# sashajenner/honours

Measured on AMD Instinct MI355X. Metric: raw-signal MB/s (compress+decompress), higher is better.
Workload: dtype u16

## Files before the change

### honours_amd/csrc/press_huffman.hip

```cpp

#include "press_internal.h"
#include "press_packed.h"
#include <cstddef>
#include <type_traits>

namespace ph {

#ifdef HUF_STAMPS
__device__ unsigned long long g_hstamp[32];
#define HSTAMP_DECL                                             \
	unsigned long long hs_t = __builtin_amdgcn_s_memtime(); \
	unsigned long long hs_acc[8] = { 0, 0, 0, 0, 0, 0, 0, 0 }
#define HSTAMP(i)                                                              \
	do {     \
		__builtin_amdgcn_sched_barrier(0);                             \
		const unsigned long long hs_n = __builtin_amdgcn_s_memtime(); \
		hs_acc[(i) & 7] += hs_n - hs_t;                                \
		hs_t = hs_n;                                                   \
		__builtin_amdgcn_sched_barrier(0);                             \
	} while (0)
#define HSTAMP_FLUSH(base)                                                     \
	do {                                                                   \
		if ((threadIdx.x & 63) == 0)                                   \
			for (int hs_i = 0; hs_i < 8; hs_i++)                   \
				atomicAdd(&g_hstamp[(base) + hs_i], hs_acc[hs_i]); \
	} while (0)
#else
#define HSTAMP_DECL
#define HSTAMP(i)
#define HSTAMP_FLUSH(base)
#endif

constexpr uint32_t HEND = 0xFFFFFFFFu;
constexpr uint32_t R_END = 31;
constexpr int HT = HUF_HT;

__device__ __forceinline__ uint32_t uniform(uint32_t v) { return (uint32_t) __builtin_amdgcn_readfirstlane((int) v); }
__device__ __forceinline__ bool any64(bool c) { return __builtin_amdgcn_ballot_w64(c) != 0; }

__device__ __forceinline__ uint32_t wave_scan(uint32_t v)
{
	v += (uint32_t) __builtin_amdgcn_update_dpp(0, (int) v, 0x111, 0xf, 0xf, true);
	v += (uint32_t) __builtin_amdgcn_update_dpp(0, (int) v, 0x112, 0xf, 0xf, true);
	v += (uint32_t) __builtin_amdgcn_update_dpp(0, (int) v, 0x114, 0xf, 0xf, true);
	v += (uint32_t) __builtin_amdgcn_update_dpp(0, (int) v, 0x118, 0xf, 0xf, true);
	v += (uint32_t) __builtin_amdgcn_update_dpp(0, (int) v, 0x142, 0xa, 0xf, false);
	v += (uint32_t) __builtin_amdgcn_update_dpp(0, (int) v, 0x143, 0xc, 0xf, false);
	return v;
}

__device__ __noinline__ uint32_t trie_code(const HuffDev *hd, uint32_t wnd)
{
	int node = 0;
	uint32_t l = 0;
	while (node >= 0 && hd->leaf[node] < 0 && l < 32) {
		node = hd->child[node][(wnd >> l) & 1u];
		l++;
	}
	if (node < 0 || hd->leaf[node] < 0)
		return 0;
	return (uint32_t) hd->leaf[node] | (l << 8) | (l << 24);
}

template <int RU>
struct HufGeo {
	static constexpr int OWN = 2 * RU;
	static constexpr int NDW = OWN / 32 + 1;
	static constexpr int NCOL = NDW + 1;
};

__device__ __forceinline__ uint32_t clamp_nb(int64_t v)
{
	return v <= 0 ? 0u : (v > 0x7FFFFFFF ? 0x7FFFFFFFu : (uint32_t) v);
}

#ifndef HUF_NO_NT
__device__ __forceinline__ uint4 ld16_pay(const uint8_t *p)
{
	typedef uint32_t u32x4_u __attribute__((ext_vector_type(4), aligned(1)));
	const u32x4_u v = __builtin_nontemporal_load(reinterpret_cast<const u32x4_u *>(p));
	return make_uint4(v.x, v.y, v.z, v.w);
}
__device__ __forceinline__ uint32_t ld4_pay(const uint8_t *p)
{
	typedef uint32_t __attribute__((aligned(1))) u32_u;
	return __builtin_nontemporal_load(reinterpret_cast<const u32_u *>(p));
}
#else
__device__ __forceinline__ uint4 ld16_pay(const uint8_t *p)
{
	uint4 v;
	__builtin_memcpy(&v, p, 16);
	return v;
}
__device__ __forceinline__ uint32_t ld4_pay(const uint8_t *p)
{
	uint32_t v;
	__builtin_memcpy(&v, p, 4);
	return v;
}
#endif

template <int NDW, int S = 64>
__device__ __forceinline__ void col_load(uint32_t *col, const uint8_t *src, int32_t rb0, int32_t lo, int32_t nby)
{
	if (rb0 >= lo && rb0 + 4 * NDW <= nby) {
		const uint8_t *q = src + rb0;
		uint4 t[NDW / 4 ? NDW / 4 : 1];
		uint32_t x[NDW % 4 ? NDW % 4 : 1];
#pragma unroll
		for (int j = 0; j < NDW / 4; j++)
			t[j] = ld16_pay(q + 16 * j);
#pragma unroll
		for (int j = 0; j < NDW % 4; j++)
			x[j] = ld4_pay(q + 4 * (NDW / 4 * 4 + j));
#pragma unroll
		for (int j = 0; j < NDW / 4; j++) {
			col[(4 * j + 0) * S] = t[j].x;
			col[(4 * j + 1) * S] = t[j].y;
			col[(4 * j + 2) * S] = t[j].z;
			col[(4 * j + 3) * S] = t[j].w;
		}
#pragma unroll
		for (int j = 0; j < NDW % 4; j++)
			col[(NDW / 4 * 4 + j) * S] = x[j];
	} else if (nby > lo) {
		uint8_t b[4 * NDW];
#pragma unroll
		for (int i = 0; i < 4 * NDW; i++) {
			const int32_t r = rb0 + i;
			b[i] = src[r < lo ? lo : (r >= nby ? nby - 1 : r)];
		}
#pragma unroll
		for (int j = 0; j < NDW; j++) {
			uint32_t x = 0;
#pragma unroll
			for (int i = 0; i < 4; i++) {
				const int32_t r = rb0 + 4 * j + i;
				x |= (r >= lo && r < nby) ? (uint32_t) b[4 * j + i] << (8 * i) : 0u;
			}
			col[j * S] = x;
		}
	} else {
#pragma unroll
		for (int j = 0; j < NDW; j++)
			col[j * S] = 0;
	}
}

__device__ __forceinline__ int32_t unzz8(uint32_t z) { return (int32_t) (z >> 1) ^ -(int32_t) (z & 1u); }

typedef __attribute__((address_space(3))) const uint32_t *lds_cu32p;
typedef __attribute__((address_space(3))) const uint16_t *lds_cu16p;
typedef __attribute__((address_space(3))) const uint8_t *lds_cu8p;
typedef __attribute__((address_space(3))) uint8_t *lds_u8p;

struct LenTabs {
	alignas(16) uint32_t alut[1 << HUF_LUT_BITS];
	alignas(16) uint16_t flut[1 << HUF_LUT_BITS];
	alignas(16) uint16_t l2ld[HUF_L2_ENTRIES];
};

template <bool TRIE, int S = 64>
__device__ __forceinline__ uint32_t len_scan(const uint32_t *col_, const LenTabs *tabs, const HuffDev *hd, uint32_t start,
					     uint32_t lim, uint32_t nb, uint32_t &cnt, uint32_t &dsum)
{
	const lds_cu32p col = (lds_cu32p) col_;
	const lds_cu32p alut = (lds_cu32p) tabs->alut;
	const lds_cu16p flut = (lds_cu16p) tabs->flut;
	const lds_cu16p l2ld = (lds_cu16p) tabs->l2ld;
	bool bad = start == HEND;
	uint32_t L = lim < nb ? lim : nb;
	if (bad)
		L = 0;
	auto long_ld = [&](uint32_t e, uint32_t wnd) -> uint32_t {
		if (TRIE && e == 0xFFFFFFFFu) {
			const uint32_t t = trie_code(hd, wnd);
			return t ? (((t >> 24) & 31u) | (((uint32_t) unzz8(t & 0xFFu) & 0xFFu) << 8)) : 0u;
		}
		const uint32_t v = l2ld[(e & 0xFFFu) + ((wnd >> HUF_LUT_BITS) & ((1u << ((e >> 12) & 15u)) - 1u))];
		return v == 0xFFFFu ? 0u : v;
	};
	constexpr uint32_t PB = 30;
	const lds_cu32p colm = col - S;
	uint32_t A = (bad ? 0u : start) + PB;
	{
		int32_t LmP = (int32_t) L - HUF_LUT_BITS + (int32_t) PB;
		uint32_t jj = (A >> 5) & 15u;
		uint32_t w0 = colm[__umul24(jj, (uint32_t) S)], w1 = colm[__umul24(jj, (uint32_t) S) + S];
		while ((int32_t) (A & 0x1FFu) <= LmP) {
			const uint32_t pp = A & 0x1FFu;
			{
				const uint32_t w2 = colm[__umul24(jj, (uint32_t) S) + 2 * S];
				const uint32_t wnd = __builtin_amdgcn_alignbit(w1, w0, A);
				const uint32_t e = *(lds_cu32p) ((lds_cu8p) alut + (wnd & (((1u << HUF_LUT_BITS) - 1u) << 2)));
				uint32_t inc = e;
				if ((int32_t) e < 0) {
					const uint32_t ld = long_ld(e, wnd >> 2);
					const uint32_t tot = ld & 0xFFu;
					inc = tot | (1u << HUF_A_CNT) | (((uint32_t) (int32_t) (int8_t) (ld >> 8) & 0x7FFFu) << HUF_A_SUM);
					if (tot - 1u >= L + PB - pp) {
						inc = 0;
						LmP = -1;
					}
				}
				A += inc;
				const uint32_t jn = (A >> 5) & 15u;
				if (jn != jj) {
					w0 = w1;
					w1 = w2;
				}
				jj = jn;
			}
		}
	}
	uint32_t p = (A & 0x1FFu) - PB;
	uint32_t c = (A >> HUF_A_CNT) & 0x7Fu;
	int32_t d = (int32_t) (A << 1) >> 17;
	for (;;) {
		const bool act = p < L;
		if (!any64(act))
			break;
		const uint32_t pp = act ? p : 0u;
		const uint32_t j = pp >> 5;
		const int r0 = (int) __umul24(j, (uint32_t) S);
		const uint32_t wnd = __builtin_amdgcn_alignbit(col[r0 + S], col[r0], pp);
		const uint32_t e = alut[wnd & ((1u << HUF_LUT_BITS) - 1u)];
		const uint32_t f = flut[wnd & ((1u << HUF_LUT_BITS) - 1u)];
		uint32_t tot = e & 15u, n = (e >> HUF_A_CNT) & 15u, len1 = f & 0xFFu;
		int32_t dall = (int32_t) (e << 1) >> 17, d1 = (int32_t) (int8_t) (f >> 8);
		bool fail = false;
		if (any64(act && (int32_t) e < 0)) {
			if (act && (int32_t) e < 0) {
				const uint32_t ld = long_ld(e, wnd);
				tot = len1 = ld & 0xFFu;
				dall = d1 = (int32_t) (int8_t) (ld >> 8);
				fail = tot == 0;
				n = 1;
			}
		}
		const bool fits = pp + tot <= L;
		const bool cut = !fits && pp + len1 > nb;
		if (act && !fail && !cut) {
			p += fits ? tot : len1;
			c += fits ? n : 1u;
			d += fits ? dall : d1;
		}
		if (act && (fail || cut)) {
			bad = true;
			L = 0;
		}
	}
	cnt = c;
	dsum = (uint32_t) d & 0xFFFFu;
	return bad ? HEND : (p >= nb && p < lim ? HEND : p);
}

__device__ __forceinline__ void wave_lds_sync()
{
	__builtin_amdgcn_fence(__ATOMIC_RELEASE, "wavefront");
	__builtin_amdgcn_wave_barrier();
	__builtin_amdgcn_fence(__ATOMIC_ACQUIRE, "wavefront");
}



#ifndef HUF_SYNC_PER_CU
#define HUF_SYNC_PER_CU 2
#endif
#ifndef HUF_RUNUP_EIGHTHS
#define HUF_RUNUP_EIGHTHS 4
#endif
constexpr int WGS = 1024;
constexpr int SYNC_S = 64;

__device__ __forceinline__ uint32_t pack_rec(uint32_t f, uint32_t c, uint32_t d)
{
	return (f == HEND ? R_END : f) | ((c & 0xFFu) << 8) | ((d & 0xFFFFu) << 16);
}

constexpr uint32_t LIST_NONE = 0xFFFFFFFFu;
constexpr uint32_t SYNC_UC = 16;

__device__ __forceinline__ void list_push(uint32_t *list, uint32_t *cnt, uint32_t cap, bool yes, uint32_t value, uint32_t lane)
{
	const unsigned long long m = __ballot(yes);
	if (!m)
		return;
	uint32_t base = 0;
	if (lane == (uint32_t) __builtin_ctzll(m))
		base = atomicAdd(cnt, (uint32_t) __popcll(m));
	base = (uint32_t) __shfl((int) base, __builtin_ctzll(m), 64);
	const uint32_t idx = base + (uint32_t) __popcll(m & ((1ull << lane) - 1ull));
	if (yes && idx < cap)
		list[idx] = value;
}

__device__ __forceinline__ void load_len_tables(const HuffDev *hd, LenTabs *t, uint32_t nthr)
{
	const uint4 *s4 = reinterpret_cast<const uint4 *>(hd->alut);
	uint4 *d4 = reinterpret_cast<uint4 *>(t->alut);
	for (uint32_t i = threadIdx.x; i < (1u << HUF_LUT_BITS) / 4; i += nthr)
		d4[i] = s4[i];
	const uint4 *f4 = reinterpret_cast<const uint4 *>(hd->flut);
	uint4 *g4 = reinterpret_cast<uint4 *>(t->flut);
	for (uint32_t i = threadIdx.x; i < (1u << HUF_LUT_BITS) / 8; i += nthr)
		g4[i] = f4[i];
	const uint4 *t4 = reinterpret_cast<const uint4 *>(hd->l2ld);
	uint4 *u4 = reinterpret_cast<uint4 *>(t->l2ld);
	for (uint32_t i = threadIdx.x; i < (uint32_t) HUF_L2_ENTRIES / 8; i += nthr)
		u4[i] = t4[i];
}


template <int RU, bool TRIE>
__global__ __launch_bounds__(WGS, 2 * HUF_SYNC_PER_CU * 2) void k_huf_sync(DecodeArgs a)
{
	constexpr int OWN = HufGeo<RU>::OWN, NDW = HufGeo<RU>::NDW;
	constexpr int RUNUP = OWN * HUF_RUNUP_EIGHTHS / 8;
	constexpr int S = SYNC_S;
	struct Lds {
		LenTabs tabs;
		uint32_t imgs[WGS / 64][(NDW + 2) * S];
	};
	__shared__ __attribute__((aligned(16))) Lds lds;
	__shared__ unsigned long long s_chunk[64];
	__shared__ uint32_t s_ticket;
	auto &imgs = lds.imgs;

	const uint32_t n = min(uniform(a.ctl->nchunks), a.max_htiles);
	const uint32_t nunits = n * (HT / 64);
	const uint32_t lane = threadIdx.x & 63;
	if (threadIdx.x == 0)
		s_ticket = 0;
	if (threadIdx.x < 64)
		s_chunk[threadIdx.x] = ~0ull;
	load_len_tables(a.huff, &lds.tabs, WGS);
	__syncthreads();
	uint32_t *img = imgs[threadIdx.x >> 6];
	for (uint32_t i = lane; i < 2 * S; i += 64)
		img[NDW * S + i] = 0;
	uint32_t *col = img + lane;
	HSTAMP_DECL;
	for (;;) {
		uint32_t u = 0;
		if (lane == 0) {
			const uint32_t t = atomicAdd(&s_ticket, 1u);
			const uint32_t c = t / SYNC_UC, slot = t % SYNC_UC;
			unsigned long long *cs = &s_chunk[c & 63u];
			if (slot == 0) {
				u = atomicAdd(&a.ctl->sunits, SYNC_UC);
				__hip_atomic_store(cs, ((unsigned long long) c << 32) | u, __ATOMIC_RELAXED, __HIP_MEMORY_SCOPE_WORKGROUP);
			} else {
				unsigned long long v;
				do {
					v = __hip_atomic_load(cs, __ATOMIC_RELAXED, __HIP_MEMORY_SCOPE_WORKGROUP);
				} while ((uint32_t) (v >> 32) != c);
				u = (uint32_t) v + slot;
			}
		}
		u = uniform(u);
		if (u >= nunits)
			break;
		HSTAMP(0);
		const uint32_t k = u / (HT / 64);
		const uint32_t tid = (u % (HT / 64)) * 64 + lane;
		const HufTile *dp = a.htiles + k;
		const uint32_t nbits_t = uniform(dp->nbits);
		const uint32_t t = uniform(dp->t_last) & 0x7FFFFFFFu;
		const uint8_t *src = a.in + dp->src;
		const int32_t nby = (int32_t) ((nbits_t + 7) >> 3);
		const bool exact = t == 0 && tid < 64;

		wave_lds_sync();
		col_load<NDW, S>(col, src, (int32_t) tid * (OWN / 8), 0, nby);
		wave_lds_sync();
		HSTAMP(1);
		const uint32_t nb = clamp_nb((int64_t) nbits_t - (int64_t) tid * OWN);

		uint32_t f, c0, c, dz, dv;
		{
			const uint32_t g = len_scan<TRIE, S>(col, &lds.tabs, a.huff, (uint32_t) (OWN - RUNUP), OWN, nb, c0, dz);
			const uint32_t gl = (uint32_t) __shfl_up((int) g, 1, 64);
			f = gl == HEND ? HEND : gl - OWN;
			if (gl == HEND && nb > 0)
				f = 0;
			if (lane == 0)
				f = nb > 0 ? 0u : HEND;
		}
		HSTAMP(2);
		const uint32_t e = len_scan<TRIE, S>(col, &lds.tabs, a.huff, f, OWN, nb, c, dv);
		HSTAMP(3);
		const uint32_t e8 = e == HEND ? R_END : e - OWN;
		const uint32_t cw = wave_scan(c), dw = wave_scan(dv);
		const uint32_t f8 = f == HEND ? R_END : f;
		const uint32_t pe8 = (uint32_t) __shfl_up((int) e8, 1, 64);
		const bool broken = lane ? f8 != pe8 : !exact;
		const unsigned long long bm = __ballot(broken);
		a.hrec[(uint64_t) k * HT + tid] = pack_rec(f, c, dv);
		a.hend[(uint64_t) k * HT + tid] = (uint8_t) e8;
		if (lane == 63) {
			a.hwave[u] = make_uint2(cw, dw & 0xFFFFu);
			a.hbits[u] = bm;
		}
		HSTAMP(4);
	}
	HSTAMP_FLUSH(0);
}

constexpr int LIST_WG = 1024;
__global__ __launch_bounds__(LIST_WG) void k_huf_list(DecodeArgs a)
{
	__shared__ uint32_t s_w[LIST_WG / 64];
	__shared__ uint32_t s_base;
	const uint32_t n = min(uniform(a.ctl->nchunks), a.max_htiles) * (HT / 64);
	const uint32_t u = blockIdx.x * LIST_WG + threadIdx.x;
	const uint32_t lane = threadIdx.x & 63, w = threadIdx.x >> 6;
	unsigned long long bm = u < n ? a.hbits[u] : 0ull;
	const uint32_t cnt = (uint32_t) __popcll(bm);
	const uint32_t inc = wave_scan(cnt);
	if (lane == 63)
		s_w[w] = inc;
	__syncthreads();
	uint32_t before = 0, total = 0;
#pragma unroll
	for (int i = 0; i < LIST_WG / 64; i++) {
		const uint32_t x = s_w[i];
		if (i < (int) w)
			before += x;
		total += x;
	}
	if (threadIdx.x == 0)
		s_base = total ? atomicAdd(&a.ctl->ticket2, total) : 0u;
	__syncthreads();
	uint32_t at = s_base + before + inc - cnt;
	while (bm) {
		const uint32_t b = (uint32_t) __builtin_ctzll(bm);
		bm &= bm - 1;
		if (at < a.hlist_cap)
			a.hlist[at] = u * 64 + b;
		at++;
	}
}

#ifndef HUF_FIX_WG
#define HUF_FIX_WG 1024
#endif
constexpr int FIX_WG = HUF_FIX_WG;
template <int RU, bool TRIE>
__global__ __launch_bounds__(FIX_WG) void k_huf_fix(DecodeArgs a, int round, int last)
{
	constexpr int OWN = HufGeo<RU>::OWN, NDW = HufGeo<RU>::NDW, NCOL = HufGeo<RU>::NCOL;
	struct Lds {
		LenTabs tabs;
		uint32_t imgs[FIX_WG / 64][NCOL * 64 + 64];
	};
	__shared__ __attribute__((aligned(16))) Lds lds;
	auto &imgs = lds.imgs;

	const uint32_t *in_list = a.hlist + (round & 1 ? a.hlist_cap : 0u);
	uint32_t *out_list = a.hlist + (round & 1 ? 0u : a.hlist_cap);
	const uint32_t *in_cnt = round ? &a.ctl->lists[round - 1] : &a.ctl->ticket2;
	uint32_t *out_cnt = &a.ctl->lists[round];
	const uint32_t n = min(uniform(*in_cnt), a.hlist_cap);
	if ((uint32_t) FIX_WG * blockIdx.x >= n)
		return;
	const uint32_t lane = threadIdx.x & 63;
	load_len_tables(a.huff, &lds.tabs, FIX_WG);
	__syncthreads();
	uint32_t *col = imgs[threadIdx.x >> 6] + lane;
	for (uint32_t i0 = FIX_WG * blockIdx.x + (threadIdx.x & ~63u); i0 < n; i0 += (uint32_t) FIX_WG * gridDim.x) {
		uint32_t ent = i0 + lane < n ? in_list[i0 + lane] : LIST_NONE;
		if (ent != LIST_NONE && (a.hrec[ent] & 0xFFu) == a.hend[ent - 1])
			ent = LIST_NONE;
		const bool mine = ent != LIST_NONE;
		const uint64_t g = mine ? ent : 1u;
		const uint32_t k = (uint32_t) (g / HT), tid = (uint32_t) (g % HT);
		const HufTile *dp = a.htiles + k;
		const uint32_t nbits_t = mine ? dp->nbits : 0u;
		wave_lds_sync();
		if (mine)
			col_load<NDW>(col, a.in + dp->src, (int32_t) tid * (OWN / 8), 0, (int32_t) ((nbits_t + 7) >> 3));
		wave_lds_sync();
		const uint32_t pe = mine ? a.hend[g - 1] : R_END;
		const uint32_t old_e = mine ? a.hend[g] : R_END;
		uint32_t c2, d2;
		const uint32_t e2 = len_scan<TRIE>(col, &lds.tabs, a.huff, (!mine || pe == R_END) ? HEND : pe, OWN,
					     clamp_nb((int64_t) nbits_t - (int64_t) tid * OWN), c2, d2);
		const uint32_t e8 = e2 == HEND ? R_END : e2 - OWN;
		bool next = false;
		if (mine) {
			const uint32_t old = a.hrec[g];
			a.hrec[g] = pack_rec(pe == R_END ? HEND : pe, c2, d2);
			const long long dc = (long long) (int32_t) (c2 - ((old >> 8) & 0xFFu));
			const unsigned long long dd = (d2 - (old >> 16)) & 0xFFFFu;
			if (dc != 0 || dd != 0)
				atomicAdd(reinterpret_cast<unsigned long long *>(a.hwave + (uint64_t) k * (HT / 64) + (tid >> 6)),
					  (dd << 32) + (unsigned long long) dc);
			if (e8 != old_e) {
				a.hend[g] = (uint8_t) e8;
				const bool more = tid + 1 < HT || !(dp->t_last >> 31);
				next = more && (uint64_t) tid * OWN + OWN < nbits_t;
			}
		}
		list_push(out_list, out_cnt, a.hlist_cap, next, (uint32_t) g + 1, lane);
		if (last && next)
			atomicMin(&a.hmin[dp->read], (uint32_t) g + 1);
	}
}

template <int RU, bool TRIE>
__global__ __launch_bounds__(64) void k_huf_serial(DecodeArgs a)
{
	constexpr int OWN = HufGeo<RU>::OWN, NDW = HufGeo<RU>::NDW, NCOL = HufGeo<RU>::NCOL;
	struct Lds {
		LenTabs tabs;
		uint32_t img[NCOL * 64 + 64];
	};
	__shared__ __attribute__((aligned(16))) Lds lds;
	auto &img = lds.img;

	const uint32_t r = blockIdx.x;
	const uint32_t g0 = uniform(a.hmin[r]);
	if (g0 == 0xFFFFFFFFu)
		return;
	const uint32_t lane = threadIdx.x;
	const uint32_t k0 = uniform(a.hread[2 * r]), nt = uniform(a.hread[2 * r + 1]);
	load_len_tables(a.huff, &lds.tabs, 64);
	uint32_t *col = img + lane;
	const uint64_t gend = (uint64_t) (k0 + nt) * HT;
	for (uint64_t g = g0; g < gend; g++) {
		const uint32_t k = (uint32_t) (g / HT), tid = (uint32_t) (g % HT);
		const HufTile *dp = a.htiles + k;
		const uint32_t nbits_t = uniform(dp->nbits);
		if ((uint64_t) tid * OWN >= nbits_t)
			break;
		const uint32_t pe = uniform((uint32_t) __hip_atomic_load(a.hend + g - 1, __ATOMIC_RELAXED, __HIP_MEMORY_SCOPE_AGENT));
		const uint32_t rec = uniform(__hip_atomic_load(a.hrec + g, __ATOMIC_RELAXED, __HIP_MEMORY_SCOPE_AGENT));
		if ((rec & 0xFFu) == pe)
			continue;
		wave_lds_sync();
		if (lane == 0)
			col_load<NDW>(col, a.in + dp->src, (int32_t) tid * (OWN / 8), 0, (int32_t) ((nbits_t + 7) >> 3));
		wave_lds_sync();
		uint32_t c2, d2;
		const uint32_t e2 = len_scan<TRIE>(col, &lds.tabs, a.huff, (lane || pe == R_END) ? HEND : pe, OWN,
					     clamp_nb((int64_t) nbits_t - (int64_t) tid * OWN), c2, d2);
		if (lane == 0) {
			a.hrec[g] = pack_rec(pe == R_END ? HEND : pe, c2, d2);
			atomicAdd(reinterpret_cast<unsigned long long *>(a.hwave + (uint64_t) k * (HT / 64) + (tid >> 6)),
				  ((unsigned long long) ((d2 - (rec >> 16)) & 0xFFFFu) << 32) +
					  (unsigned long long) (long long) (int32_t) (c2 - ((rec >> 8) & 0xFFu)));
			__hip_atomic_store(a.hend + g, (uint8_t) (e2 == HEND ? R_END : e2 - OWN), __ATOMIC_RELAXED, __HIP_MEMORY_SCOPE_AGENT);
		}
		__builtin_amdgcn_fence(__ATOMIC_RELEASE, "agent");
	}
}

__device__ __forceinline__ uint32_t unzz16(uint32_t z) { return ((z >> 1) ^ (0u - (z & 1u))) & 0xFFFFu; }

__device__ __forceinline__ void keys_below2(const uint32_t *pos, uint32_t nex, uint32_t ka, uint32_t kb, uint32_t &ea, uint32_t &eb)
{
	uint32_t la = 0, lb = 0;
	for (uint32_t step = nex ? 1u << (31 - __builtin_clz(nex)) : 0u; step; step >>= 1) {
		const uint32_t ia = la + step - 1, ib = lb + step - 1;
		const uint32_t pa = ia < nex ? pos[ia] : 0u, pb = ib < nex ? pos[ib] : 0u;
		if (ia < nex && pa - ia < ka)
			la += step;
		if (ib < nex && pb - ib < kb)
			lb += step;
	}
	ea = la;
	eb = lb;
}

template <int RU>
__global__ __launch_bounds__(HT) void k_huf_chain(DecodeArgs a)
{
	constexpr uint32_t UB = 64 * HufGeo<RU>::OWN / 8;
	constexpr uint32_t UPT = HT / 64;
	__shared__ uint32_t s_w[HT / 64], s_wd[HT / 64];
	__shared__ unsigned long long s_cum;

	const uint32_t r = blockIdx.x;
	const uint32_t tid = threadIdx.x;
	const uint32_t k0 = uniform(a.hread[2 * r]), nt = uniform(a.hread[2 * r + 1]);
	if (!nt)
		return;
	const uint32_t nu = nt * UPT;
	const uint2 *hw = a.hwave + (uint64_t) k0 * UPT;
	if (tid == 0)
		s_cum = 0;
	__syncthreads();
	{
		uint64_t c = 0;
		for (uint32_t u = tid; u < nu; u += HT)
			c += hw[u].x;
		if (c)
			atomicAdd(&s_cum, (unsigned long long) c);
	}
	const uint32_t want = uniform(a.htiles[k0].want);
	const uint32_t nex = uniform(a.meta[r].nex);
	const uint64_t o0 = a.htiles[k0].low;
	uint32_t *val = a.ex_val + o0;
	const uint32_t *pos = a.ex_pos + o0;
	uint32_t xcum = 0;
	for (uint32_t b = 0; b < nex; b += HT) {
		const uint32_t e = b + tid;
		const uint32_t z = e < nex ? (val[e] & 0xFFFFu) : 0u;
		const uint32_t dl = e < nex ? unzz16(z) : 0u;
		const uint32_t inc = wave_scan(dl);
		if ((tid & 63) == 63)
			s_w[tid >> 6] = inc;
		__syncthreads();
		uint32_t before = 0, total = 0;
#pragma unroll
		for (int w2 = 0; w2 < HT / 64; w2++) {
			const uint32_t x = s_w[w2];
			if (w2 < (int) (tid >> 6))
				before += x;
			total += x;
		}
		if (e < nex)
			val[e] = z | (((xcum + before + inc - dl) & 0xFFFFu) << 16);
		xcum += total;
		__syncthreads();
	}
	__syncthreads();
	const uint64_t cumall = s_cum;
	const uint32_t nlow = cumall < want ? (uint32_t) cumall : want;
	const bool fused = nlow >= 1 && (nex == 0 || pos[nex - 1] < nlow + nex);
	const uint32_t zd0 = uniform(a.meta[r].zd0) & 0xFFFFu, q = uniform(a.meta[r].q);
	const uint64_t src0 = a.htiles[k0].src;
	const int64_t nby0 = (int64_t) ((a.htiles[k0].nbits + 7u) >> 3);
	uint64_t cum = 0;
	uint32_t dcum = 0;
	for (uint32_t b = 0; b < nu; b += HT) {
		const uint32_t u = b + tid;
		uint32_t c = 0, dt = 0;
		if (u < nu) {
			const uint2 w = hw[u];
			c = w.x;
			dt = w.y & 0xFFFFu;
		}
		const uint32_t inc = wave_scan(c);
		const uint32_t dinc = wave_scan(dt);
		if ((tid & 63) == 63) {
			s_w[tid >> 6] = inc;
			s_wd[tid >> 6] = dinc;
		}
		__syncthreads();
		uint32_t before = 0, total = 0, dbefore = 0, dtotal = 0;
#pragma unroll
		for (int w2 = 0; w2 < HT / 64; w2++) {
			const uint32_t x = s_w[w2], y = s_wd[w2];
			if (w2 < (int) (tid >> 6)) {
				before += x;
				dbefore += y;
			}
			total += x;
			dtotal += y;
		}
		if (u < nu) {
			const uint64_t ob = cum + before + inc - c;
			const uint32_t L0 = ob > 0xFFFFFFFFull ? 0xFFFFFFFFu : (uint32_t) ob;
			const uint32_t quota = L0 >= want ? 0u : (c < want - L0 ? c : want - L0);
			const uint32_t L1 = L0 + quota;
			uint32_t Ea = 0, Eb = 0;
			if (fused && quota) {
				keys_below2(pos, nex, L0, L1, Ea, Eb);
				if (L1 == nlow)
					Eb = nex;
			}
			uint32_t bz = zd0;
			if (L0) {
				bz = unzz16(zd0) + ((dcum + dbefore + dinc - dt) & 0xFFFFu);
				if (Ea) {
					const uint32_t pv = val[Ea - 1];
					bz += (pv >> 16) + unzz16(pv & 0xFFFFu);
				}
				bz &= 0xFFFFu;
			}
			const uint64_t src = src0 + (uint64_t) u * UB;
			const int64_t nby = nby0 - (int64_t) u * UB;
			const uint32_t nbyc = nby <= 0 ? 0u : (nby > (int64_t) HUF_U_NBY ? HUF_U_NBY : (uint32_t) nby);
			uint4 *d = reinterpret_cast<uint4 *>(a.hunit + (uint64_t) k0 * UPT + u);
			d[0] = make_uint4((uint32_t) src, (uint32_t) (src >> 32) | (bz << 16), (uint32_t) o0, (uint32_t) (o0 >> 32));
			d[1] = make_uint4(L0, quota | (nbyc << 14) | ((q & 15u) << 26) | (fused ? 1u << 30 : 0u), Ea, Eb - Ea);
		}
		cum += total;
		dcum += dtotal;
		__syncthreads();
	}
	static_assert(HUF_U_QUOTA >= 64u * 255u, "a unit's quota");
	if (tid == 0) {
		a.meta[r].nlow = nlow;
		if (fused)
			a.hread[2 * r + 1] = nt | HUF_FUSED;
	}
}


constexpr uint32_t EMIT_STG = 4096;

template <bool TRIE>
__device__ __forceinline__ void emit_codes(const uint32_t *col_, const uint32_t *lut_, const uint16_t *lut2_,
					   const HuffDev *hd, uint32_t p, uint32_t nmine, uint8_t *wp_)
{
	const lds_cu32p col = (lds_cu32p) col_;
	const lds_cu8p lut = (lds_cu8p) lut_;
	const lds_cu16p lut2 = (lds_cu16p) lut2_;
	auto long_entry = [&](uint32_t e, uint32_t wnd) -> uint32_t {
		if (TRIE && e == 0xFFFFFFFFu) {
			const uint32_t t = trie_code(hd, wnd);
			return t ? ((t & 0xFFFFFF00u) | ((uint32_t) unzz8(t & 0xFFu) & 0xFFu)) : 0u;
		}
		const uint32_t e2 = lut2[(e & 0xFFFu) + ((wnd >> HUF_LUT_BITS) & ((1u << ((e >> 12) & 15u)) - 1u))];
		return e2 == 0xFFFFu ? 0u : (((uint32_t) unzz8(e2 & 0xFFu) & 0xFFu) | (e2 & 0x1F00u) | ((e2 & 0x1F00u) << 16));
	};
	typedef lds_u8p WP;
	WP w = (WP) wp_;
	const WP wend = w + nmine;
	WP wlim = nmine ? wend - 1 : w;
	constexpr uint32_t PB = 30;
	const lds_cu32p colm = col - 64;
	uint32_t pp = p + PB;
	uint32_t jj = pp >> 5;
	uint32_t w0 = colm[__umul24(jj, 64u)], w1 = colm[__umul24(jj, 64u) + 64];
	while (w < wlim) {
		{
			const uint32_t w2 = colm[__umul24(jj, 64u) + 128];
			const uint32_t wnd = __builtin_amdgcn_alignbit(w1, w0, pp);
			uint32_t e = *(lds_cu32p) (lut + (wnd & (((1u << HUF_LUT_BITS) - 1u) << 2)));
			if (e >= HUF_LONG)
				e = long_entry(e, wnd >> 2);
			w[0] = (uint8_t) e;
			w[1] = (uint8_t) (e >> 16);
			w += 1u + ((e >> 29) & 1u);
			pp += (e >> 8) & 0x1Fu;
			const uint32_t jn = pp >> 5;
			if (jn != jj) {
				w0 = w1;
				w1 = w2;
			}
			jj = jn;
		}
	}
	if (w < wend) {
		const uint32_t wnd = __builtin_amdgcn_alignbit(w1, w0, pp);
		uint32_t e = *(lds_cu32p) (lut + (wnd & (((1u << HUF_LUT_BITS) - 1u) << 2)));
		if (e >= HUF_LONG)
			e = long_entry(e, wnd >> 2);
		w[0] = (uint8_t) e;
	}
}


__device__ __forceinline__ uint32_t lower_bound_u32(const uint32_t *p, uint32_t n, uint32_t key)
{
	uint32_t lo = 0, hi = n;
	while (lo < hi) {
		const uint32_t mid = (lo + hi) >> 1;
		if (p[mid] < key)
			lo = mid + 1;
		else
			hi = mid;
	}
	return lo;
}

template <typename LOWAT, typename BELOW, typename POSAT, typename VALAT>
__device__ __forceinline__ void gather8(LOWAT lowat, BELOW below, POSAT posat, VALAT valat, uint32_t zd0, uint32_t i0,
					uint32_t Ia, uint32_t Ib, uint32_t e_first, uint32_t e_cnt, uint32_t v[4])
{
	v[0] = v[1] = v[2] = v[3] = 0;
	const uint32_t lo = i0 > Ia ? i0 : Ia;
	const uint32_t hi = i0 + 8 < Ib ? i0 + 8 : Ib;
	if (lo >= hi)
		return;
	const uint32_t uf = lo ? lo - 1 : 0;
	uint32_t k = below(uf);
	uint32_t l = uf - e_first - k;
	uint32_t nextpos = k < e_cnt ? posat(k) : 0xFFFFFFFFu;
#pragma unroll
	for (int h = 0; h < 8; h++) {
		const uint32_t i = i0 + h;
		if (i >= lo && i < hi) {
			uint32_t dl;
			if (i == 0) {
				dl = unzz16(zd0);
			} else if (i - 1 == nextpos) {
				dl = unzz16(valat(k) & 0xFFFFu);
				k++;
				nextpos = k < e_cnt ? posat(k) : 0xFFFFFFFFu;
			} else {
				dl = lowat(l) & 0xFFFFu;
				l++;
			}
			v[h >> 1] |= dl << (16 * (h & 1));
		}
	}
}

struct EmitRead {
	const uint32_t *pos, *val;
	int16_t *out;
	uint32_t zd0, q;
};

constexpr uint32_t EMIT_ALIGN = 8;

__device__ __forceinline__ void expand8s(uint2 dd, uint32_t v[4])
{
	typedef short i16x2 __attribute__((ext_vector_type(2)));
	const i16x2 eight = { 8, 8 };
	const uint32_t t[4] = { __builtin_amdgcn_perm(0, dd.x, 0x010c000c), __builtin_amdgcn_perm(0, dd.x, 0x030c020c),
				__builtin_amdgcn_perm(0, dd.y, 0x010c000c), __builtin_amdgcn_perm(0, dd.y, 0x030c020c) };
#pragma unroll
	for (int h = 0; h < 4; h++)
		v[h] = __builtin_bit_cast(uint32_t, __builtin_bit_cast(i16x2, t[h]) >> eight);
}

struct EmitPlan {
	uint32_t L0, L1;
	uint32_t Ea, ecnt;
	uint32_t Ia, Ib;
	uint32_t base;
	uint32_t pe;
};

template <bool BIG>
__device__ __forceinline__ void emit_samples16(const uint8_t *src, uint32_t *exl_, const EmitRead &R, const EmitPlan &P,
					       uint32_t lane)
{
	typedef __attribute__((address_space(3))) uint32_t *lds_u32p;
	const uint32_t L0 = P.L0, L1 = P.L1, Ea = P.Ea, ecnt = P.ecnt, Ia = P.Ia, Ib = P.Ib, pe = P.pe;
	uint32_t base = P.base;
	const lds_u32p exl = (lds_u32p) exl_;
	if (!BIG) {
		uint32_t ve = 0;
		if (ecnt != 0 && lane < ecnt)
			ve = R.val[Ea + lane];
		exl[lane] = pe;
		exl[64 + lane] = ve;
		wave_lds_sync();
	}
	auto ex_below = [&](uint32_t key) -> uint32_t {
		if (BIG)
			return uniform(lower_bound_u32(R.pos + Ea, ecnt, key));
		return (uint32_t) __popcll(__ballot(pe < key));
	};
	auto below = [&](uint32_t key) -> uint32_t {
		if (BIG)
			return lower_bound_u32(R.pos + Ea, ecnt, key);
		uint32_t k = 0;
#pragma unroll
		for (uint32_t st = 32; st; st >>= 1)
			k += exl[k + st - 1] < key ? st : 0u;
		return k + (exl[k] < key ? 1u : 0u);
	};
	auto posat = [&](uint32_t k) -> uint32_t { return BIG ? R.pos[Ea + k] : exl[k]; };
	auto valat = [&](uint32_t k) -> uint32_t { return BIG ? R.val[Ea + k] : exl[64 + k]; };
	const bool shift = uniform(R.q) != 0;
	const u16x2 qq = { (unsigned short) R.q, (unsigned short) R.q };
	const uint32_t *s32 = reinterpret_cast<const uint32_t *>(src);
	for (uint32_t g = Ia & ~(EMIT_ALIGN - 1); g < Ib; g += 1024) {
		const uint32_t i0 = g + lane * 16;
		const uint32_t e0 = ex_below(g ? g - 1 : 0u), e1 = ex_below(g + 1023);
		const bool plain = e0 == e1 && g != 0;
		const bool ragged = g < Ia || g + 1024 > Ib;
		uint32_t v[8];
		if (plain) {
			const bool any = i0 + 16 > Ia && i0 < Ib;
			const int32_t o = any ? (int32_t) (i0 - 1 - Ea - e0 - L0) : 0;
			const int32_t j = o >> 2;
			const uint32_t sh = (uint32_t) (o & 3) * 8u;
			const uint32_t d0 = s32[j], d1 = s32[j + 1], d2 = s32[j + 2], d3 = s32[j + 3], d4 = s32[j + 4];
			uint2 da = make_uint2(__builtin_amdgcn_alignbit(d1, d0, sh), __builtin_amdgcn_alignbit(d2, d1, sh));
			uint2 db = make_uint2(__builtin_amdgcn_alignbit(d3, d2, sh), __builtin_amdgcn_alignbit(d4, d3, sh));
			if (g < Ia) {
				auto mask8 = [&](uint2 &dd, uint32_t ia) {
					const uint32_t lo = Ia > ia ? (Ia - ia < 8 ? Ia - ia : 8u) : 0u;
					const uint64_t m = lo >= 8 ? 0ull : ~((1ull << (8 * lo)) - 1ull);
					dd.x &= (uint32_t) m;
					dd.y &= (uint32_t) (m >> 32);
				};
				mask8(da, i0);
				mask8(db, i0 + 8);
			}
			expand8s(da, v);
			expand8s(db, v + 4);
		} else {
			auto lowat = [&](uint32_t l) -> uint32_t { return (l >= L0 && l < L1) ? (uint32_t) (int32_t) (int8_t) src[l - L0] : 0u; };
			gather8(lowat, below, posat, valat, R.zd0, i0, Ia, Ib, Ea, ecnt, v);
			gather8(lowat, below, posat, valat, R.zd0, i0 + 8, Ia, Ib, Ea, ecnt, v + 4);
		}
		const uint32_t ta = lane_prefix8(v) & 0xFFFFu;
		const uint32_t tb = lane_prefix8(v + 4) & 0xFFFFu;
		const uint32_t tot = (ta + tb) & 0xFFFFu;
		const uint32_t inc = wave_incl_scan_dpp(tot);
		const uint32_t ba = (base + inc - tot) & 0xFFFFu, bb = (ba + ta) & 0xFFFFu;
		const uint32_t ba2 = ba | (ba << 16), bb2 = bb | (bb << 16);
#pragma unroll
		for (int h = 0; h < 4; h++) {
			v[h] = pk_add16(v[h], ba2);
			v[4 + h] = pk_add16(v[4 + h], bb2);
		}
		if (shift) {
#pragma unroll
			for (int h = 0; h < 8; h++)
				v[h] = __builtin_bit_cast(uint32_t, __builtin_bit_cast(u16x2, v[h]) << qq);
		}
#if defined(EMIT_ABL) && EMIT_ABL == 1
		if (R.q == 0x7FFFFFFFu)
#endif
#pragma unroll
		for (int hh = 0; hh < 2; hh++) {
			const uint32_t ia = i0 + 8 * hh;
			if (!ragged || (ia >= Ia && ia + 8 <= Ib)) {
				typedef uint32_t u32x4 __attribute__((ext_vector_type(4)));
				const u32x4 vv = { v[4 * hh], v[4 * hh + 1], v[4 * hh + 2], v[4 * hh + 3] };
#ifdef EMIT_NT_STORES
				__builtin_nontemporal_store(vv, reinterpret_cast<u32x4 *>(R.out + ia));
#else
				*reinterpret_cast<u32x4 *>(R.out + ia) = vv;
#endif
			} else if (ia < Ib && ia + 8 > Ia) {
#pragma unroll
				for (uint32_t h = 0; h < 8; h++)
					if (ia + h >= Ia && ia + h < Ib)
						R.out[ia + h] = (int16_t) (v[4 * hh + (h >> 1)] >> (16 * (h & 1)));
			}
		}
		base += (uint32_t) __builtin_amdgcn_readlane((int) inc, 63);
	}
}

__device__ __forceinline__ uint32_t zz_bytes(uint32_t d)
{
	return ((d << 1) & 0xFEFEFEFEu) ^ (((d >> 7) & 0x01010101u) * 0xFFu);
}

#ifndef EMIT_WG
#define EMIT_WG 512
#endif
#ifndef EMIT_PER_CU
#define EMIT_PER_CU 2
#endif
constexpr int WGE = EMIT_WG;
constexpr uint32_t EMIT_UC = 16;

struct EmitStg {
	uint8_t pre[16];
	uint8_t s[WGE / 64][EMIT_STG];
	uint8_t post[32];
};

template <int RU, bool TRIE>
__global__ __launch_bounds__(WGE) void k_huf_emit(DecodeArgs a)
{
	constexpr int OWN = HufGeo<RU>::OWN, NDW = HufGeo<RU>::NDW, NCOL = HufGeo<RU>::NDW;
	constexpr uint32_t EW = WGE / 64;
	struct Lds {
		alignas(16) uint32_t lut[1 << HUF_LUT_BITS];
		alignas(16) uint16_t lut2[HUF_L2_ENTRIES];
		uint32_t img[EW][NCOL * 64];
		uint32_t pad_row[2 * 64];
		alignas(16) EmitStg stg_all;
		uint32_t exl[EW][128];
	};
	__shared__ __attribute__((aligned(16))) Lds lds;
	auto &lut = lds.lut;
	auto &lut2 = lds.lut2;
	auto &img = lds.img;
	auto &pad_row = lds.pad_row;
	auto &stg_all = lds.stg_all;
	__shared__ unsigned long long s_chunk[64];
	__shared__ uint32_t s_ticket;

	const uint32_t lane = threadIdx.x & 63;
	const uint32_t wv = threadIdx.x >> 6;
	const uint32_t ntiles = min(uniform(a.ctl->nchunks), a.max_htiles);
	const uint32_t nunits = ntiles * (HT / 64);
	if (threadIdx.x == 0) {
		pad_row[0] = 0;
		s_ticket = 0;
	}
	if (threadIdx.x < 64)
		s_chunk[threadIdx.x] = ~0ull;
	{
		const uint4 *s4 = reinterpret_cast<const uint4 *>(a.huff->lut32);
		uint4 *d4 = reinterpret_cast<uint4 *>(lut);
		for (uint32_t i = threadIdx.x; i < (1u << HUF_LUT_BITS) / 4; i += WGE)
			d4[i] = s4[i];
		const uint4 *t4 = reinterpret_cast<const uint4 *>(a.huff->lut2);
		uint4 *u4 = reinterpret_cast<uint4 *>(lut2);
		for (uint32_t i = threadIdx.x; i < (uint32_t) HUF_L2_ENTRIES / 8; i += WGE)
			u4[i] = t4[i];
	}
// ... 326 lines not shown
```

Before: 796,000.

## Process two adjacent Huffman subtiles per lane in sync kernel with register payload

The Huffman sync pass now has each lane decode two consecutive subtiles. It loads their payload into registers once with vectorized loads, then stages each half into LDS before running the length scans. Only the second subtile needs a runup scan, so the number of scans per pair drops from four to three, and the records are written as packed uint2/uint16 values. Per-64-thread wave and bitmask outputs are rebuilt with shuffles and bit interleaving. The chain kernel also gains a validation path: when the code-count total falls short of the expected count, it walks the Huffman trie serially to detect invalid codes and refuses fusion, which adds work on that path.

```diff
diff --git a/honours_amd/csrc/press_huffman.hip b/honours_amd/csrc/press_huffman.hip
--- a/honours_amd/csrc/press_huffman.hip
+++ b/honours_amd/csrc/press_huffman.hip
@@ -145,6 +145,52 @@
 #pragma unroll
 		for (int j = 0; j < NDW; j++)
 			col[j * S] = 0;
+	}
+}
+
+template <int NP>
+__device__ __forceinline__ void pay_load(uint32_t (&r)[NP], const uint8_t *src, int32_t rb0, int32_t nby)
+{
+	if (rb0 + 4 * NP <= nby) {
+		const uint8_t *q = src + rb0;
+		uint4 t[NP / 4 ? NP / 4 : 1];
+		uint32_t x[NP % 4 ? NP % 4 : 1];
+#pragma unroll
+		for (int j = 0; j < NP / 4; j++)
+			t[j] = ld16_pay(q + 16 * j);
+#pragma unroll
+		for (int j = 0; j < NP % 4; j++)
+			x[j] = ld4_pay(q + 4 * (NP / 4 * 4 + j));
+#pragma unroll
+		for (int j = 0; j < NP / 4; j++) {
+			r[4 * j + 0] = t[j].x;
+			r[4 * j + 1] = t[j].y;
+			r[4 * j + 2] = t[j].z;
+			r[4 * j + 3] = t[j].w;
+		}
+#pragma unroll
+		for (int j = 0; j < NP % 4; j++)
+			r[NP / 4 * 4 + j] = x[j];
+	} else if (nby >= 4) {
+		uint32_t d[NP];
+#pragma unroll
+		for (int j = 0; j < NP; j++) {
+			const int32_t p = rb0 + 4 * j;
+			d[j] = ld4_pay(src + (p < nby - 4 ? p : nby - 4));
+		}
+#pragma unroll
+		for (int j = 0; j < NP; j++) {
+			const int32_t over = rb0 + 4 * j - (nby - 4);
+			r[j] = over <= 0 ? d[j] : (over < 4 ? d[j] >> (8 * over) : 0u);
+		}
+	} else {
+		uint32_t x = 0;
+		if (rb0 == 0)
+			for (int32_t i = 0; i < nby; i++)
+				x |= (uint32_t) src[i] << (8 * i);
+#pragma unroll
+		for (int j = 0; j < NP; j++)
+			r[j] = j ? 0u : x;
 	}
 }
 
@@ -313,12 +359,35 @@
 }
 
 
+template <int NDW, int S>
+__device__ __forceinline__ void col_put(uint32_t *col, const uint32_t *r)
+{
+	wave_lds_sync();
+#pragma unroll
+	for (int j = 0; j < NDW; j++)
+		col[j * S] = r[j];
+	wave_lds_sync();
+}
+
+__device__ __forceinline__ unsigned long long spread32(uint32_t x)
+{
+	unsigned long long v = x;
+	v = (v | v << 16) & 0x0000FFFF0000FFFFull;
+	v = (v | v << 8) & 0x00FF00FF00FF00FFull;
+	v = (v | v << 4) & 0x0F0F0F0F0F0F0F0Full;
+	v = (v | v << 2) & 0x3333333333333333ull;
+	v = (v | v << 1) & 0x5555555555555555ull;
+	return v;
+}
+
 template <int RU, bool TRIE>
 __global__ __launch_bounds__(WGS, 2 * HUF_SYNC_PER_CU * 2) void k_huf_sync(DecodeArgs a)
 {
 	constexpr int OWN = HufGeo<RU>::OWN, NDW = HufGeo<RU>::NDW;
+	constexpr int W = OWN / 32, NP = 2 * W + 1;
 	constexpr int RUNUP = OWN * HUF_RUNUP_EIGHTHS / 8;
 	constexpr int S = SYNC_S;
+	constexpr uint32_t UP = HT / 128;
 	struct Lds {
 		LenTabs tabs;
 		uint32_t imgs[WGS / 64][(NDW + 2) * S];
@@ -329,7 +398,7 @@
 	auto &imgs = lds.imgs;
 
 	const uint32_t n = min(uniform(a.ctl->nchunks), a.max_htiles);
-	const uint32_t nunits = n * (HT / 64);
+	const uint32_t nunits = n * UP;
 	const uint32_t lane = threadIdx.x & 63;
 	if (threadIdx.x == 0)
 		s_ticket = 0;
@@ -363,47 +432,59 @@
 		if (u >= nunits)
 			break;
 		HSTAMP(0);
-		const uint32_t k = u / (HT / 64);
-		const uint32_t tid = (u % (HT / 64)) * 64 + lane;
+		const uint32_t k = u / UP;
+		const uint32_t tid = (u % UP) * 128 + 2 * lane;
 		const HufTile *dp = a.htiles + k;
 		const uint32_t nbits_t = uniform(dp->nbits);
 		const uint32_t t = uniform(dp->t_last) & 0x7FFFFFFFu;
 		const uint8_t *src = a.in + dp->src;
 		const int32_t nby = (int32_t) ((nbits_t + 7) >> 3);
-		const bool exact = t == 0 && tid < 64;
-
-		wave_lds_sync();
-		col_load<NDW, S>(col, src, (int32_t) tid * (OWN / 8), 0, nby);
-		wave_lds_sync();
+		const bool exact = t == 0 && u % UP == 0;
+
+		uint32_t pay[NP];
+		pay_load<NP>(pay, src, (int32_t) tid * (OWN / 8), nby);
+		col_put<NDW, S>(col, pay + W);
 		HSTAMP(1);
-		const uint32_t nb = clamp_nb((int64_t) nbits_t - (int64_t) tid * OWN);
-
-		uint32_t f, c0, c, dz, dv;
+		const uint32_t nbA = clamp_nb((int64_t) nbits_t - (int64_t) tid * OWN);
+		const uint32_t nbB = clamp_nb((int64_t) nbits_t - (int64_t) (tid + 1) * OWN);
+
+		uint32_t fA, c0, cA, cB, dz, dA, dB;
 		{
-			const uint32_t g = len_scan<TRIE, S>(col, &lds.tabs, a.huff, (uint32_t) (OWN - RUNUP), OWN, nb, c0, dz);
+			const uint32_t g = len_scan<TRIE, S>(col, &lds.tabs, a.huff, (uint32_t) (OWN - RUNUP), OWN, nbB, c0, dz);
 			const uint32_t gl = (uint32_t) __shfl_up((int) g, 1, 64);
-			f = gl == HEND ? HEND : gl - OWN;
-			if (gl == HEND && nb > 0)
-				f = 0;
+			fA = gl == HEND ? HEND : gl - OWN;
+			if (gl == HEND && nbA > 0)
+				fA = 0;
 			if (lane == 0)
-				f = nb > 0 ? 0u : HEND;
+				fA = nbA > 0 ? 0u : HEND;
 		}
 		HSTAMP(2);
-		const uint32_t e = len_scan<TRIE, S>(col, &lds.tabs, a.huff, f, OWN, nb, c, dv);
+		col_put<NDW, S>(col, pay);
+		const uint32_t eA = len_scan<TRIE, S>(col, &lds.tabs, a.huff, fA, OWN, nbA, cA, dA);
 		HSTAMP(3);
-		const uint32_t e8 = e == HEND ? R_END : e - OWN;
-		const uint32_t cw = wave_scan(c), dw = wave_scan(dv);
-		const uint32_t f8 = f == HEND ? R_END : f;
-		const uint32_t pe8 = (uint32_t) __shfl_up((int) e8, 1, 64);
-		const bool broken = lane ? f8 != pe8 : !exact;
-		const unsigned long long bm = __ballot(broken);
-		a.hrec[(uint64_t) k * HT + tid] = pack_rec(f, c, dv);
-		a.hend[(uint64_t) k * HT + tid] = (uint8_t) e8;
-		if (lane == 63) {
-			a.hwave[u] = make_uint2(cw, dw & 0xFFFFu);
-			a.hbits[u] = bm;
-		}
+		uint32_t fB = eA == HEND ? HEND : eA - OWN;
+		if (eA == HEND && nbB > 0)
+			fB = 0;
+		col_put<NDW, S>(col, pay + W);
+		const uint32_t eB = len_scan<TRIE, S>(col, &lds.tabs, a.huff, fB, OWN, nbB, cB, dB);
 		HSTAMP(4);
+		const uint32_t eA8 = eA == HEND ? R_END : eA - OWN, eB8 = eB == HEND ? R_END : eB - OWN;
+		const uint32_t cw = wave_scan(cA + cB), dw = wave_scan(dA + dB);
+		const uint32_t fA8 = fA == HEND ? R_END : fA, fB8 = fB == HEND ? R_END : fB;
+		const uint32_t pe8 = (uint32_t) __shfl_up((int) eB8, 1, 64);
+		const unsigned long long bmA = __ballot(lane ? fA8 != pe8 : !exact), bmB = __ballot(fB8 != eA8);
+		const uint64_t ri = (uint64_t) k * HT + tid;
+		*reinterpret_cast<uint2 *>(a.hrec + ri) = make_uint2(pack_rec(fA, cA, dA), pack_rec(fB, cB, dB));
+		*reinterpret_cast<uint16_t *>(a.hend + ri) = (uint16_t) (eA8 | (eB8 << 8));
+		const uint32_t cw31 = (uint32_t) __shfl((int) cw, 31, 64), dw31 = (uint32_t) __shfl((int) dw, 31, 64);
+		if ((lane & 31u) == 31u) {
+			const bool hi = lane == 63;
+			const uint32_t uu = 2 * u + (hi ? 1u : 0u);
+			a.hwave[uu] = make_uint2(hi ? cw - cw31 : cw, (hi ? dw - dw31 : dw) & 0xFFFFu);
+			a.hbits[uu] = hi ? spread32((uint32_t) (bmA >> 32)) | spread32((uint32_t) (bmB >> 32)) << 1
+					 : spread32((uint32_t) bmA) | spread32((uint32_t) bmB) << 1;
+		}
+		HSTAMP(5);
 	}
 	HSTAMP_FLUSH(0);
 }
@@ -463,6 +544,10 @@
 	const uint32_t *in_cnt = round ? &a.ctl->lists[round - 1] : &a.ctl->ticket2;
 	uint32_t *out_cnt = &a.ctl->lists[round];
 	const uint32_t n = min(uniform(*in_cnt), a.hlist_cap);
+#ifdef HUF_STAMPS
+	if (blockIdx.x == 0 && threadIdx.x == 0)
+		g_hstamp[16 + (round & 7)] = n;
+#endif
 	if ((uint32_t) FIX_WG * blockIdx.x >= n)
 		return;
 	const uint32_t lane = threadIdx.x & 63;
@@ -581,6 +666,7 @@
 	constexpr uint32_t UPT = HT / 64;
 	__shared__ uint32_t s_w[HT / 64], s_wd[HT / 64];
 	__shared__ unsigned long long s_cum;
+	__shared__ uint32_t s_stop, s_refuse;
 
 	const uint32_t r = blockIdx.x;
 	const uint32_t tid = threadIdx.x;
@@ -589,8 +675,11 @@
 		return;
 	const uint32_t nu = nt * UPT;
 	const uint2 *hw = a.hwave + (uint64_t) k0 * UPT;
-	if (tid == 0)
+	if (tid == 0) {
 		s_cum = 0;
+		s_stop = 0xFFFFFFFFu;
+		s_refuse = 0;
+	}
 	__syncthreads();
 	{
 		uint64_t c = 0;
@@ -629,7 +718,40 @@
 	__syncthreads();
 	const uint64_t cumall = s_cum;
 	const uint32_t nlow = cumall < want ? (uint32_t) cumall : want;
-	const bool fused = nlow >= 1 && (nex == 0 || pos[nex - 1] < nlow + nex);
+	if (cumall < want) {
+		constexpr uint32_t OWN = HufGeo<RU>::OWN;
+		const uint64_t nbits0 = a.htiles[k0].nbits;
+		const uint64_t nsub64 = (nbits0 + OWN - 1) / OWN;
+		const uint32_t nsub = nsub64 < (uint64_t) nt * HT ? (uint32_t) nsub64 : nt * HT;
+		const uint8_t *he = a.hend + (uint64_t) k0 * HT;
+		for (uint32_t i = tid; i < nsub; i += HT)
+			if (he[i] == R_END) {
+				atomicMin(&s_stop, i);
+				break;
+			}
+		__syncthreads();
+		if (tid == 0 && s_stop != 0xFFFFFFFFu) {
+			const uint32_t f = a.hrec[(uint64_t) k0 * HT + s_stop] & 0xFFu;
+			if (f != R_END) {
+				const HuffDev *hd = a.huff;
+				const uint8_t *pay = a.in + a.htiles[k0].src;
+				uint64_t p = (uint64_t) s_stop * OWN + f;
+				int node = 0;
+				for (uint32_t i = 0; i < OWN + 64 && p < nbits0; i++, p++) {
+					node = hd->child[node][(pay[p >> 3] >> (p & 7)) & 1u];
+					if (node < 0) {
+						s_refuse = 1;
+						break;
+					}
+					if (hd->leaf[node] >= 0)
+						node = 0;
+				}
+			}
+		}
+		__syncthreads();
+	}
+	const bool refused = s_refuse != 0;
+	const bool fused = !refused && nlow >= 1 && (nex == 0 || pos[nex - 1] < nlow + nex);
 	const uint32_t zd0 = uniform(a.meta[r].zd0) & 0xFFFFu, q = uniform(a.meta[r].q);
 	const uint64_t src0 = a.htiles[k0].src;
 	const int64_t nby0 = (int64_t) ((a.htiles[k0].nbits + 7u) >> 3);
@@ -695,6 +817,8 @@
 	static_assert(HUF_U_QUOTA >= 64u * 255u, "a unit's quota");
 	if (tid == 0) {
 		a.meta[r].nlow = nlow;
+		if (refused)
+			a.meta[r].status = 1;
 		if (fused)
 			a.hread[2 * r + 1] = nt | HUF_FUSED;
 	}
```

Result: faster. 832,800 (median of 6 runs) (+4.6%).
